# johanngerberding/voxelnet-pytorch

Measured on AMD Instinct MI355X. Metric: point-clouds/sec fwd+bwd, KITTI car voxel grid, batch=2, higher is better.
Workload: dtype bf16; 1 GPU; KITTI car config (voxel 0.2x0.2x0.4 m, grid 10x400x352, T=35), batch=2 per GPU, fwd+bwd train step (BASELINE configs[1]); global_batch=2, points_per_frame=19861, parallelism=dp1, launch_mode=eager+native-executor+one-call-step

## Files before the change

include/voxelnet_hip.h:

```cpp
#ifndef VOXELNET_HIP_H
#define VOXELNET_HIP_H

#include <stddef.h>
#include <stdint.h>

#ifdef __cplusplus
extern "C" {
#endif

#define VN_OK 0
#define VN_EINVAL (-1)
#define VN_EUNSUPPORTED (-2)
#define VN_EWORKSPACE (-3)

typedef enum { VN_F32 = 0, VN_BF16 = 1,
               VN_F32X3 = 2,
               VN_F32X3S = 3 } vnDtype;

typedef void *vnStream;

int vn_abi_version(void);
const char *vn_build_info(void);
const char *vn_build_id(void);

// ... 72 lines not shown
    int32_t Dr, Hr, Wr;
    int32_t Cs;
    int32_t src_wrap;
    int32_t Cr;
    int32_t kD, kH, kW;
    int32_t mulD, mulH, mulW;
    int32_t tmulD, tmulH, tmulW;
    int32_t padD, padH, padW;
    int32_t divD, divH, divW;
    int64_t src_sB, src_sD, src_sH, src_sW;
    int64_t out_sB, out_sD, out_sH, out_sW;
} vnConv;

int64_t vn_conv_stats_slab_rows(const vnConv *geom);
int vn_conv_gather_gemm(const void *src, const void *w_packed ,
                        const float *bias , void *out, vnDtype out_dtype,
                        const vnConv *geom, int32_t accumulate, float *stats_slab,
                        vnStream stream);
int32_t vn_conv_plan_id(const vnConv *geom);

size_t vn_conv_wgrad_workspace_bytes(const vnConv *geom, int32_t split, int64_t n_rows);
int vn_conv_wgrad(const void *src , const void *rows , float *dw_packed,
                  const vnConv *geom, int32_t split, void *workspace, size_t workspace_bytes,
                  vnStream stream);
int32_t vn_conv_wgrad_plan_id(const vnConv *geom, int32_t split, int64_t n_rows);
int vn_conv_wgrad_partials(const void *src, const void *rows, const vnConv *geom, int32_t split,
                           const int64_t *row_list, int64_t n_rows, void *workspace,
                           size_t workspace_bytes, int32_t *chunks, vnStream stream);
int vn_conv_wgrad_partials_split_pass(const void *src, const void *rows, const vnConv *geom, int32_t pass, void *workspace,
                                      size_t workspace_bytes, int32_t *chunks, vnStream stream);

int vn_conv_dgrad_bn_bwd(const void *src, const void *w_packed, void *out, vnDtype out_dtype, const vnConv *geom,
                         const void *bn_y, vnDtype bn_y_dtype, const float *bn_stats, float *slab, vnStream stream);
int vn_conv_gather_gemm_rows(const void *src, const void *w_packed, const float *bias, void *out,
                             vnDtype out_dtype, const vnConv *geom, const int64_t *row_list,
                             int64_t row_cap, const int32_t *row_count, int32_t out_linear,
                             float *stats_slab, vnStream stream);
int vn_conv_wgrad_rows(const void *src, const void *rows, float *dw_packed, const vnConv *geom,
                       const int64_t *row_list, int64_t n_rows, void *workspace, size_t workspace_bytes,
                       vnStream stream);
int vn_conv_wgrad_partials_counted(const void *src, const void *rows, const vnConv *geom, const int64_t *row_list,
                                   int64_t row_cap, const int32_t *row_count, void *workspace, size_t workspace_bytes,
                                   int32_t *chunks, vnStream stream);
size_t vn_active_sites_workspace_bytes(const vnConv *geom);
int vn_active_sites(const int64_t *coord, int64_t K, const vnConv *geom, void *workspace,
                    size_t workspace_bytes, int64_t *list, int64_t cap, int32_t *count, vnStream stream);
int vn_voxel_index_grid(const int64_t *coord, int64_t K, int32_t B, int32_t D, int32_t H, int32_t W,
                        int32_t *grid , vnStream stream);
int64_t vn_rulebook_slab_rows(int64_t cap);
int vn_rulebook_combine(const float *P, const int32_t *index_grid, const int64_t *list, int64_t cap,
                        const int32_t *count, const vnConv *geom, const float *bias, void *y,
                        vnDtype y_dtype, float *stats_slab, vnStream stream);
int vn_fill_rows(void *y, vnDtype dtype, int64_t M, int32_t C, int64_t stride, const float *values,
                 vnStream stream);

int vn_pack_weight(const float *w, int32_t c_out, int32_t c_in, int32_t taps, int32_t mode,
                   int32_t split3, int32_t cin_fold, void *packed, vnDtype packed_dtype,
                   vnStream stream);
int vn_unpack_wgrad(const float *dw_packed, int32_t c_out, int32_t c_in, int32_t taps,
                    int32_t mode, int32_t cin_fold, float *dw, vnStream stream);
typedef struct vnPackJob {
    const float *w;
    void *packed;
    int32_t c_out, c_in, taps, mode, split3, cin_fold;
    int32_t packed_dtype;
    int32_t pad_;
// ... 474 lines not shown
```

voxelnet-pytorch_amd/csrc/abi.hip:

```cpp
#include "common.h"
#include <mutex>
#include <stdio.h>
#include <stdlib.h>
#include <string.h>

#include "build_id.h"

extern "C" int vn_abi_version(void) { return 4; }
extern "C" const char *vn_build_id(void) { return VN_BUILD_ID; }

namespace {
const char *const KNOBS[] = {"VN_DUP", "VN_EARLY_DECONV", "VN_FUSE_BWD_REDUCE", "VN_GG_CONFIG", "VN_HEADS_STREAM", "VN_M0_BN", "VN_PATCH", "VN_PATCH2D",
                               "VN_SKIP", "VN_WGP_BLOCKS", "VN_WGRAD_PATCH", "VN_WG_BLOCKS"};
constexpr int NKNOBS = sizeof(KNOBS) / sizeof(KNOBS[0]);
}

int vn_knob(const char *name, int dflt) {
    for (int i = 0; i < NKNOBS; ++i)
        if (!strcmp(KNOBS[i], name)) {
            const char *e = getenv(name);
            return e && *e ? atoi(e) : dflt;
        }
    static std::mutex mu;
    static const char *seen[16];
    static int nseen = 0;
    std::lock_guard<std::mutex> lock(mu);
    for (int i = 0; i < nseen; ++i)
        if (!strcmp(seen[i], name)) return dflt;
    if (nseen < 16) seen[nseen++] = name;
    fprintf(stderr, "libvoxelnet_hip: vn_knob(\"%s\") is not in the KNOBS table of csrc/abi.hip — the default %d is used and the "
                    "environment is NOT read\n", name, dflt);
    return dflt;
}

extern "C" const char *vn_build_info(void) {
    static char buf[1536];
    static std::once_flag once;
    std::call_once(once, [] {
        size_t n = (size_t)snprintf(buf, sizeof(buf), "libvoxelnet_hip gfx950 (CDNA4) abi %d build " VN_BUILD_ID " " __DATE__ " " __TIME__, vn_abi_version());
        bool any = false;
        for (int i = 0; i < NKNOBS && n + 64 < sizeof(buf); ++i) {
            const char *e = getenv(KNOBS[i]);
            if (!e || !*e) continue;
            n += (size_t)snprintf(buf + n, sizeof(buf) - n, "%s%s=%.24s", any ? " " : " overrides: ", KNOBS[i], e);
            any = true;
        }
// ... 4 lines not shown
```

voxelnet-pytorch_amd/csrc/conv.hip:

```cpp
#include "common.h"

namespace {

constexpr int GG_MAX_TAPS = 32;
constexpr int GG_MAX_CLASSES = 16;
constexpr uint32_t GG_OOB = 0xFFFFF000u;
constexpr uint32_t GG_MAX_WINDOW = 0xFFFFE000u;

struct GGClass {
    int32_t tap_begin, ntaps;
    int32_t nD, nH, nW;
    int32_t qD, qH, qW;
    int32_t ooffD, ooffH, ooffW;
    int32_t offD[4], offH[4], offW[4];
};
struct GGTap {
    int32_t id, ih, iw, widx;
};
struct GGParams {
    const char *src;
    const char *w;
    const float *bias;
    char *out;
    float *stats;
// ... 873 lines not shown
                            acc[i][j] = __builtin_amdgcn_mfma_f32_16x16x32_bf16(a, bq[j], acc[i][j], 0, 0, 0);
                    }
                }
            }
            }
#ifdef VN_P2D_TRACE
            if (tr_on) {
                asm volatile("s_nop 0" ::"v"(acc[0][0]), "v"(acc[SM - 1][3]));
                P2D_STAMP(s, 4);
            }
#endif
        }
        pbuf ^= 1;
    }

    __syncthreads();
    int32_t *otab = reinterpret_cast<int32_t *>(smem);
    for (int r = threadIdx.x; r < BM; r += NT) {
        const int py = r / TW, px = r - py * TW;
        const int qh = y0 + py, qw = x0 + px;
        int32_t off = -1;
        if (qh < cl.qH && qw < cl.qW) {
            const int od = qd * p.omulD + cl.ooffD, oh = qh * p.omulH + cl.ooffH, ow = qw * p.omulW + cl.ooffW;
            if (od < p.Do && oh < p.Ho && ow < p.Wo)
                off = (int32_t)((int64_t)b * p.oB + (int64_t)od * p.oD + (int64_t)oh * p.oH + (int64_t)ow * p.oW);
        }
        otab[r] = off;
    }
    __syncthreads();
    if (p.bn_y) gg_store<WM, WN, SM, true>(p, acc, smem, otab, tile, n0, wm, wn, lane);
    else gg_store<WM, WN, SM>(p, acc, smem, otab, tile, n0, wm, wn, lane);
}

inline int floordiv(int a, int b) { return (a >= 0) ? a / b : -((-a + b - 1) / b); }
inline int posmod(int a, int b) { int r = a % b; return r < 0 ? r + b : r; }

struct AxisClass {
    int r;
    int q;
    int n;
    int tap[4];
    int off[4];
};

int axis_classes(int R, int k, int mul, int tmul, int pad, int div, AxisClass *out, int *mul_out, int *omul_out) {
    if (div == 1) {
        AxisClass c{};
        c.r = 0; c.q = R; c.n = k;
        for (int t = 0; t < k; ++t) { c.tap[t] = t; c.off[t] = t * tmul - pad; }
        out[0] = c;
        *mul_out = mul; *omul_out = 1;
        return 1;
    }
    int nc = 0;
    for (int r = 0; r < div && r < R; ++r) {
        AxisClass c{};
        c.r = r; c.q = (R - r + div - 1) / div; c.n = 0;
        for (int t = 0; t < k; ++t) {
            const int num = r + t * tmul - pad;
            if (posmod(num, div) == 0) { c.tap[c.n] = t; c.off[c.n] = floordiv(num, div); ++c.n; }
        }
        out[nc++] = c;
    }
    *mul_out = 1; *omul_out = div;
    return nc;
}
// ... 71 lines not shown
    constexpr size_t lds = 2 * ((size_t)((PROWS + 7) / 8 + NW - 1) / NW * NW * 1024) + NSB * (size_t)(64 * WN) * 128;
    static const hipError_t attr = hipFuncSetAttribute(reinterpret_cast<const void *>(&k_conv_patch2d<WM, WN, SM, TW, NSB, F32>),
                                                       hipFuncAttributeMaxDynamicSharedMemorySize, (int)lds);
    if (attr != hipSuccess) return (int)attr;
    k_conv_patch2d<WM, WN, SM, TW, NSB, F32><<<grid, 64 * NW, lds, st>>>(p);
    return 0;
}
int patch2d_stages() {
    static const int v = vn_knob("VN_PATCH2D", 3);
    return v;
}
int launch_patch_cfg(const PatchCfg &c, bool f32, const GGParams &p, dim3 grid, hipStream_t st) {
    if (c.id == 2 && p.Ds == 1 && p.nclasses == 1 && p.cls[0].nD == 1 && patch2d_stages() >= 3) {
        const GGParams &q = p;
        if (patch2d_stages() == 3 && !f32) return launch_patch2d<4, 2, 1, 16, 3, false>(q, grid, st);
        if (patch2d_stages() == 3 && f32 && q.x3) return launch_patch2d<4, 2, 1, 16, 3, true>(q, grid, st);
        if (patch2d_stages() == 3)
            return f32 ? launch_patch2d<2, 2, 2, 16, 3, true>(q, grid, st) : launch_patch2d<2, 2, 2, 16, 3, false>(q, grid, st);
        return f32 ? launch_patch2d<2, 2, 2, 16, 4, true>(q, grid, st) : launch_patch2d<2, 2, 2, 16, 4, false>(q, grid, st);
    }
    if (c.id == 3) return f32 ? launch_patch<4, 1, 3, 32, true>(p, grid, st) : launch_patch<4, 1, 3, 32, false>(p, grid, st);
    if (c.id == 2) return f32 ? launch_patch<2, 2, 2, 16, true>(p, grid, st) : launch_patch<2, 2, 2, 16, false>(p, grid, st);
    return f32 ? launch_patch<2, 2, 5, 16, true>(p, grid, st) : launch_patch<2, 2, 5, 16, false>(p, grid, st);
}

int launch_cfg(const GGConfig &c, bool f32, const GGParams &p, dim3 grid, hipStream_t st) {
    switch (c.id) {
    case 0: return f32 ? launch_gg<4, 1, 4, 2, true>(p, grid, st) : launch_gg<4, 1, 4, 2, false>(p, grid, st);
    case 1: return f32 ? launch_gg<2, 2, 4, 2, true>(p, grid, st) : launch_gg<2, 2, 4, 2, false>(p, grid, st);
    case 2: return f32 ? launch_gg<2, 2, 2, 4, true>(p, grid, st) : launch_gg<2, 2, 2, 4, false>(p, grid, st);
    case 3: return f32 ? launch_gg<4, 1, 1, 6, true>(p, grid, st) : launch_gg<4, 1, 1, 6, false>(p, grid, st);
    default: return f32 ? launch_gg<2, 2, 5, 2, true>(p, grid, st) : launch_gg<2, 2, 5, 2, false>(p, grid, st);
    }
}

struct AxisSlots {
    int n, cls[4], off[4], tap[4];
};
bool axis_slots(int k, int tmul, int pad, int div, AxisSlots *o) {
    o->n = 0;
    for (int r = 0; r < div; ++r)
        for (int t = 0; t < k; ++t) {
            const int num = r + t * tmul - pad;
            if (posmod(num, div) != 0) continue;
            if (o->n >= 4) return false;
            o->cls[o->n] = div == 1 ? -1 : r;
            o->off[o->n] = floordiv(num, div);
            o->tap[o->n] = t;
            ++o->n;
        }
    return o->n > 0;
}

}

extern "C" int vn_conv_gather_gemm_rows(const void *src, const void *w_packed, const float *bias, void *out,
                                        vnDtype out_dtype, const vnConv *g, const int64_t *row_list, int64_t row_cap,
                                        const int32_t *row_count, int32_t out_linear, float *stats_slab,
                                        vnStream stream) {
    VN_CHECK_ARG(src && w_packed && out && g && row_list && row_cap >= 0 && row_cap < (1ll << 31));
    if (row_cap == 0) return VN_OK;
    VN_CHECK_ARG(g->B > 0 && g->Ds > 0 && g->Hs > 0 && g->Ws > 0 && g->Dr > 0 && g->Hr > 0 && g->Wr > 0);
    VN_CHECK_ARG(g->kD >= 1 && g->kD <= 4 && g->kH >= 1 && g->kH <= 4 && g->kW >= 1 && g->kW <= 4);
    VN_CHECK_ARG(g->divD >= 1 && g->divH >= 1 && g->divW >= 1);
    VN_CHECK_ARG((g->divD == 1 || g->mulD == 1) && (g->divH == 1 || g->mulH == 1) && (g->divW == 1 || g->mulW == 1));
    VN_CHECK_ARG(out_dtype == VN_F32 || out_dtype == VN_BF16);
// ... 91 lines not shown
    const int64_t rows = (int64_t)g->B * g->Dr * g->Hr * g->Wr;
    return vn_ceil_div(rows, gg_config(rows, g->Cr, 1).BM);
}

extern "C" int32_t vn_conv_plan_id(const vnConv *g) {
    if (!g || g->divD < 1 || g->divH < 1 || g->divW < 1 || g->B <= 0) return -1;
    const PatchCfg pc = patch_config(g);
    if (pc.id == 2 && g->Ds == 1 && g->Dr == 1 && g->kD == 1 && g->divD == 1 && patch2d_stages() >= 3)
        return 120 + patch2d_stages();
    if (pc.id >= 0) return 100 + pc.id;
    const int64_t qd = vn_ceil_div(g->Dr, g->divD), qh = vn_ceil_div(g->Hr, g->divH), qw = vn_ceil_div(g->Wr, g->divW);
    const int nd = g->divD < g->Dr ? g->divD : g->Dr, nh = g->divH < g->Hr ? g->divH : g->Hr, nw = g->divW < g->Wr ? g->divW : g->Wr;
    return gg_config((int64_t)g->B * qd * qh * qw, g->Cr, nd * nh * nw).id;
}

static int gather_gemm_impl(const void *src, const void *w_packed, const float *bias, void *out, vnDtype out_dtype,
                            const vnConv *g, int32_t accumulate, float *stats_slab, vnStream stream, const void *bn_y,
                            vnDtype bn_y_dtype, const float *bn_stats);

extern "C" int vn_conv_gather_gemm(const void *src, const void *w_packed, const float *bias, void *out,
                                   vnDtype out_dtype, const vnConv *g, int32_t accumulate, float *stats_slab,
                                   vnStream stream) {
    return gather_gemm_impl(src, w_packed, bias, out, out_dtype, g, accumulate, stats_slab, stream, nullptr, VN_BF16, nullptr);
}

extern "C" int vn_conv_dgrad_bn_bwd(const void *src, const void *w_packed, void *out, vnDtype out_dtype, const vnConv *g,
                                    const void *bn_y, vnDtype bn_y_dtype, const float *bn_stats, float *slab,
                                    vnStream stream) {
    VN_CHECK_ARG(bn_y && bn_stats && slab && g);
    if (vn_conv_plan_id(g) != 123) return VN_EUNSUPPORTED;
    return gather_gemm_impl(src, w_packed, nullptr, out, out_dtype, g, 0, slab, stream, bn_y, bn_y_dtype, bn_stats);
}

static int gather_gemm_impl(const void *src, const void *w_packed, const float *bias, void *out, vnDtype out_dtype,
                            const vnConv *g, int32_t accumulate, float *stats_slab, vnStream stream, const void *bn_y,
                            vnDtype bn_y_dtype, const float *bn_stats) {
    VN_CHECK_ARG(src && w_packed && out && g);
    VN_CHECK_ARG(g->B > 0 && g->Ds > 0 && g->Hs > 0 && g->Ws > 0 && g->Dr > 0 && g->Hr > 0 && g->Wr > 0);
    VN_CHECK_ARG(g->kD >= 1 && g->kD <= 4 && g->kH >= 1 && g->kH <= 4 && g->kW >= 1 && g->kW <= 4);
    VN_CHECK_ARG(g->kD * g->kH * g->kW <= GG_MAX_TAPS);
    VN_CHECK_ARG(g->divD >= 1 && g->divH >= 1 && g->divW >= 1);
    VN_CHECK_ARG(g->divD == 1 || g->mulD == 1);
    VN_CHECK_ARG(g->divH == 1 || g->mulH == 1);
    VN_CHECK_ARG(g->divW == 1 || g->mulW == 1);
    VN_CHECK_ARG(out_dtype == VN_F32 || out_dtype == VN_BF16);
    VN_CHECK_ARG(!stats_slab || g->divD * g->divH * g->divW <= GG_MAX_CLASSES);
    VN_CHECK_ARG(g->dtype == VN_BF16 || g->dtype == VN_F32 || g->dtype == VN_F32X3 || g->dtype == VN_F32X3S);
    const bool f32 = g->dtype != VN_BF16;
    const int esz = f32 ? 4 : 2, bke = 128 / esz, align_e = 16 / esz;
    (void)bke;
    if (g->Cs <= 0 || (g->Cs % align_e) || g->Cr <= 0 || (g->Cr & 3)) return VN_EUNSUPPORTED;
    if (g->src_wrap != 0) return VN_EUNSUPPORTED;
    if (g->divD * g->divH * g->divW > GG_MAX_CLASSES) return VN_EUNSUPPORTED;
    if (((g->src_sB | g->src_sD | g->src_sH | g->src_sW) & (align_e - 1)) != 0) return VN_EUNSUPPORTED;
    if (((g->out_sB | g->out_sD | g->out_sH | g->out_sW) & 3) != 0) return VN_EUNSUPPORTED;
    if ((reinterpret_cast<uintptr_t>(src) & 15) || (reinterpret_cast<uintptr_t>(w_packed) & 15) ||
        (reinterpret_cast<uintptr_t>(out) & 15))
        return VN_EUNSUPPORTED;

    GGParams p{};
    p.src = static_cast<const char *>(src);
    p.w = static_cast<const char *>(w_packed);
    p.bias = bias;
    p.out = static_cast<char *>(out);
    p.stats = stats_slab;
    p.bn_y = bn_y;
// ... 106 lines not shown
```

voxelnet-pytorch_amd/csrc/runtime.hip:

```cpp
#include "common.h"
#include <new>
#include <string.h>

namespace {

constexpr int NL = 23;

struct Spec {
    int dim, cin, cout, k[3], s[3], p[3];
    bool transposed;
    int cin_fold;
};

struct Rows {
    char *ptr;
    int dtype;
    int B, D, H, W, C;
    int64_t sB, sD, sH, sW;
    int64_t M() const { return (int64_t)B * D * H * W; }
};

Rows dense_rows(void *ptr, int dtype, int B, int D, int H, int W, int C, int64_t width = 0) {
    if (!width) width = C;
    return Rows{static_cast<char *>(ptr), dtype, B, D, H, W, C, (int64_t)D * H * W * width, (int64_t)H * W * width,
// ... 1011 lines not shown
                vn_dgrad_total(dy.ptr, (vnDtype)dy.dtype, B, P.odims[l][0], P.odims[l][1], P.odims[l][2], C, sp.cin, sp.k[0],
                               L[l].weight, 0, P.dtot_ws, P.dtot_ws_bytes, P.dtot, bs));
            if (box_on_side) {
                box_ev = net->next_event();
                if (!box_ev) return VN_EINVAL;
                VN_HIP(hipEventRecord(box_ev, ws));
            }
            const int64_t rs[4] = {0, 0, 0, sp.cin};
            vnConv gl = geom(dy, P.in_dims[l], C, sp.cin, sp.k, ONE, NEG, np, sp.s, rs);
            RTT(T_CONV_DGRAD, l, 2.0 * active_rows * taps * sp.cin * C, rows_bytes(dy) + 2.0 * active_rows * sp.cin * P.esz, ls,
                vn_conv_gather_gemm_rows(dy.ptr, P.wp_d[l], nullptr, P.dx[l].ptr, (vnDtype)P.dx[l].dtype, cx(P, gl), P.alist, P.acap,
                                         P.acount, 1, nullptr, ls));
            return VN_OK;
        }
        Rows dx = P.dx[l];
        if (l == 0) {
            if (!d_input) return VN_OK;
            dx = dense_rows(d_input, P.adt, B, cfg->D, cfg->H, cfg->W, 128);
        }
        const int64_t os[4] = {dx.sB, dx.sD, dx.sH, dx.sW};
        vnConv gd = sp.transposed ? geom(dy, P.in_dims[l], C, sp.cin, sp.k, sp.s, ONE, sp.p, ONE, os)
                                  : geom(dy, P.in_dims[l], C, sp.cin, sp.k, ONE, NEG, np, sp.s, os);
        const bool below_plain = l >= 2 && l - 1 != L_M2 && l - 1 != L_D1 && l - 1 != L_D2 && l - 1 != L_D3 && l != L_D1 &&
                                 l != L_D2 && l != L_D3 && !P.spec[l - 1].transposed;
        if (fuse_bwd_reduce_on() && single_call && !accumulate && !on_side && below_plain && vn_conv_plan_id(cx(P, gd)) == 123 &&
            P.y[l - 1].sB == dx.sB && P.y[l - 1].sD == dx.sD && P.y[l - 1].sH == dx.sH && P.y[l - 1].sW == dx.sW &&
            vn_conv_stats_slab_rows(cx(P, gd)) <= P.bslab_rows[l - 1]) {
            RTT(T_CONV_DGRAD, l, layer_flops(sp, P.in_dims[l], P.odims[l], B), rows_bytes(dy) + 2.0 * rows_bytes(dx), ls,
                vn_conv_dgrad_bn_bwd(dy.ptr, P.wp_d[l], dx.ptr, (vnDtype)dx.dtype, cx(P, gd), P.y[l - 1].ptr, (vnDtype)P.y[l - 1].dtype,
                                     P.stats[l - 1], P.bslab[l - 1], ls));
            fused_rows[l - 1] = vn_conv_stats_slab_rows(cx(P, gd));
            return VN_OK;
        }
        RTT(T_CONV_DGRAD, l, layer_flops(sp, P.in_dims[l], P.odims[l], B), rows_bytes(dy) + rows_bytes(dx), ls,
            vn_conv_gather_gemm(dy.ptr, P.wp_d[l], nullptr, dx.ptr, (vnDtype)dx.dtype, cx(P, gd), accumulate ? 1 : 0, nullptr, ls));
        return VN_OK;
    };
    static const int early_on = vn_knob("VN_EARLY_DECONV", 1);
    const bool early = early_on && ws != hs && seg_begin == 0 && seg_end == NL + 1;
    hipEvent_t ev_d2 = nullptr, ev_d1 = nullptr;
    if (early) {
        if (!heads_forked) RT(fork());
        RT(do_layer(L_D2, wstream, true, false));
        ev_d2 = net->next_event();
        if (!ev_d2) return VN_EINVAL;
        VN_HIP(hipEventRecord(ev_d2, ws));
        RT(do_layer(L_D1, wstream, true, false));
        ev_d1 = net->next_event();
        if (!ev_d1) return VN_EINVAL;
        VN_HIP(hipEventRecord(ev_d1, ws));
    }
    const bool bucket_ev = cfg->bucket_events && ws != hs && seg_begin == 0 && seg_end == NL + 1;
    int u_done = 0, z_done = 0;
    auto bucket_done = [&](int b) -> int {
        RT(flush());
            if (b == 3 && m0_on_main) RT(fork());
        RTT(T_UNPACK, -1, 0.0, unpack_bytes(unpack + u_done, nu - u_done), wstream, vn_unpack_wgrads_batch(unpack + u_done, nu - u_done, wstream));
        RT(after_unpack(u_done, nu, wstream));
        u_done = nu;
        if (zj.n > z_done) {
            ZeroJobs part{};
            part.n = zj.n - z_done;
            for (int i = 0; i < part.n; ++i) { part.ptr[i] = zj.ptr[z_done + i]; part.len[i] = zj.len[z_done + i]; }
            RTT(T_MISC, -1, 0.0, 0.0, wstream, zero_many(part, ws));
            z_done = zj.n;
        }
// ... 145 lines not shown
```

voxelnet-pytorch_amd/voxelnet_amd/_lib.py:

```python
import ctypes
import os

import torch

_HERE = os.path.dirname(os.path.abspath(__file__))
LIB_PATH = os.environ.get("VN_LIB_PATH") or os.path.join(_HERE, "lib", "libvoxelnet_hip.so")

c_i32, c_i64, c_f32, c_vp, c_sz = ctypes.c_int32, ctypes.c_int64, ctypes.c_float, ctypes.c_void_p, ctypes.c_size_t

VN_F32, VN_BF16 = 0, 1
VN_F32X3S = 3


class VnGrid(ctypes.Structure):
    _fields_ = [("D", c_i32), ("H", c_i32), ("W", c_i32),
                ("vz", c_f32), ("vy", c_f32), ("vx", c_f32),
                ("ox", c_f32), ("oy", c_f32), ("oz", c_f32), ("T", c_i32)]


class VnConv(ctypes.Structure):
    _fields_ = [(n, c_i32) for n in (
        "dtype", "B", "Ds", "Hs", "Ws", "Dr", "Hr", "Wr", "Cs", "src_wrap", "Cr", "kD", "kH", "kW",
        "mulD", "mulH", "mulW", "tmulD", "tmulH", "tmulW", "padD", "padH", "padW",
        "divD", "divH", "divW")] + [(n, c_i64) for n in (
# ... 162 lines not shown
    "vn_vfe_workspace_bytes": (c_sz, [c_i64, c_i32]),
    "vn_vfe_fwd": (c_i32, [c_vp, c_i64, c_i32, _P(VnVfeWeights), c_i32, c_f32, c_f32, c_vp, c_vp, c_vp, c_sz, c_vp]),
    "vn_vfe_fwd_rows": (c_i32, [c_vp, c_i64, c_i32, _P(VnVfeWeights), c_i32, c_f32, c_f32, c_vp, c_vp, c_vp, c_vp, c_sz, c_vp]),
    "vn_vfe_bwd": (c_i32, [c_vp, c_i64, c_i32, _P(VnVfeWeights), c_vp, c_vp, _P(VnVfeGrads), c_vp, c_sz, c_i32, c_vp]),
    "vn_scatter_dense_fwd": (c_i32, [c_vp, c_vp, c_i64, c_i32, c_i32, c_i32, c_i32, c_i32, c_vp, c_i32, c_i32,
                                     c_i32, c_vp]),
    "vn_scatter_dense_update": (c_i32, [c_vp, c_vp, c_i64, c_i32, c_i32, c_i32, c_i32, c_i32, c_vp, c_i32, c_i32,
                                        c_i32, c_vp]),
    "vn_scatter_dense_bwd": (c_i32, [c_vp, c_i32, c_vp, c_i64, c_i32, c_i32, c_i32, c_i32, c_i32, c_vp, c_vp]),
    "vn_conv_gather_gemm": (c_i32, [c_vp, c_vp, c_vp, c_vp, c_i32, _P(VnConv), c_i32, c_vp, c_vp]),
    "vn_net_workspace_bytes": (c_sz, [_P(VnNetConfig), c_i64]),
    "vn_net_tensor_info": (c_i32, [_P(VnNetConfig), c_i64, c_i32, c_i32, _P(VnNetTensorInfo)]),
    "vn_net_create": (c_i32, [_P(c_vp)]),
    "vn_net_destroy": (c_i32, [c_vp]),
    "vn_net_step": (c_i32, [c_vp, _P(VnNetConfig), _P(VnStep)]),
    "vn_net_timing_begin": (c_i32, [c_vp, c_i32]),
    "vn_net_timing_read": (c_i32, [c_vp, c_vp, c_i32, _P(c_i32)]),
    "vn_net_forward": (c_i32, [c_vp, _P(VnNetConfig), _P(VnLayerParams), c_vp, c_vp, c_vp, c_vp, c_vp, c_i64, c_vp, c_sz, c_vp,
                               c_vp, c_vp, c_vp]),
    "vn_net_wait_bucket": (c_i32, [c_vp, c_i32, c_vp]),
    "vn_net_prepare": (c_i32, [c_vp, _P(VnNetConfig), _P(VnLayerParams), c_vp, c_vp, c_i64, c_vp, c_sz, c_vp]),
    "vn_voxel_index_grid": (c_i32, [c_vp, c_i64, c_i32, c_i32, c_i32, c_i32, c_vp, c_vp]),
    "vn_rulebook_slab_rows": (c_i64, [c_i64]),
    "vn_rulebook_combine": (c_i32, [c_vp, c_vp, c_vp, c_i64, c_vp, _P(VnConv), c_vp, c_vp, c_i32, c_vp, c_vp]),
    "vn_net_backward": (c_i32, [c_vp, _P(VnNetConfig), _P(VnLayerParams), c_vp, c_vp, c_vp, c_vp, c_vp, c_vp, c_vp, c_i64,
                                c_vp, c_sz, _P(VnLayerGrads), c_vp, c_vp, c_vp, c_i32, c_i32, c_vp, c_vp]),
    "vn_conv_stats_slab_rows": (c_i64, [_P(VnConv)]),
    "vn_conv_plan_id": (c_i32, [_P(VnConv)]),
    "vn_conv_wgrad_plan_id": (c_i32, [_P(VnConv), c_i32, c_i64]),
    "vn_bn_finalize_slab": (c_i32, [c_vp, c_i64, c_i64, c_i32, c_vp, c_vp, c_vp, c_vp, c_vp, c_f32, c_f32, c_vp, c_vp]),
    "vn_conv_wgrad_workspace_bytes": (c_sz, [_P(VnConv), c_i32, c_i64]),
    "vn_conv_wgrad": (c_i32, [c_vp, c_vp, c_vp, _P(VnConv), c_i32, c_vp, c_sz, c_vp]),
    "vn_conv_dgrad_bn_bwd": (c_i32, [c_vp, c_vp, c_vp, c_i32, _P(VnConv), c_vp, c_i32, c_vp, c_vp, c_vp]),
    "vn_conv_gather_gemm_rows": (c_i32, [c_vp, c_vp, c_vp, c_vp, c_i32, _P(VnConv), c_vp, c_i64, c_vp, c_i32, c_vp, c_vp]),
    "vn_conv_wgrad_partials": (c_i32, [c_vp, c_vp, _P(VnConv), c_i32, c_vp, c_i64, c_vp, c_sz, c_vp, c_vp]),
    "vn_conv_wgrad_rows": (c_i32, [c_vp, c_vp, c_vp, _P(VnConv), c_vp, c_i64, c_vp, c_sz, c_vp]),
    "vn_conv_wgrad_partials_split_pass": (c_i32, [c_vp, c_vp, _P(VnConv), c_i32, c_vp, c_sz, c_vp, c_vp]),
    "vn_active_sites_workspace_bytes": (c_sz, [_P(VnConv)]),
    "vn_active_sites": (c_i32, [c_vp, c_i64, _P(VnConv), c_vp, c_sz, c_vp, c_i64, c_vp, c_vp]),
    "vn_fill_rows": (c_i32, [c_vp, c_i32, c_i64, c_i32, c_i64, c_vp, c_vp]),
    "vn_pack_weight": (c_i32, [c_vp, c_i32, c_i32, c_i32, c_i32, c_i32, c_i32, c_vp, c_i32, c_vp]),
    "vn_unpack_wgrad": (c_i32, [c_vp, c_i32, c_i32, c_i32, c_i32, c_i32, c_vp, c_vp]),
    "vn_bn_stats": (c_i32, [c_vp, c_i32, c_i64, c_i32, c_i64, c_i32, c_vp, c_vp, c_vp]),
    "vn_bn_finalize": (c_i32, [c_vp, c_i64, c_i32, c_i32, c_vp, c_vp, c_vp, c_vp, c_vp, c_i32, c_f32, c_f32, c_vp,
                               c_vp]),
    "vn_bn_apply": (c_i32, [c_vp, c_i32, c_i64, c_i64, c_i32, c_vp, c_i32, c_vp, c_i32, c_i64, c_i64, c_vp]),
    "vn_bn_bwd_reduce": (c_i32, [c_vp, c_i32, c_i64, c_vp, c_i32, c_i64, c_i64, c_i32, c_vp, c_i32, c_vp, c_vp]),
    "vn_bn_bwd_finalize": (c_i32, [c_vp, c_i64, c_i32, c_i32, c_vp, c_vp, c_vp, c_vp, c_vp, c_vp]),
    "vn_bn_bwd_slab_rows": (c_i64, [c_i64, c_i32]),
    "vn_bn_bwd_reduce_slab": (c_i32, [c_vp, c_i32, c_i64, c_vp, c_i32, c_i64, c_i64, c_i32, c_vp, c_i32, c_vp, c_vp]),
    "vn_bn_bwd_finalize_slab": (c_i32, [c_vp, c_i64, c_i64, c_i32, c_vp, c_vp, c_vp, c_vp, c_vp, c_vp]),
    "vn_bn_bwd_apply": (c_i32, [c_vp, c_i32, c_i64, c_vp, c_i32, c_i64, c_i64, c_i32, c_vp, c_vp, c_i32, c_vp,
                                c_i32, c_i64, c_i64, c_vp]),
    "vn_bn_apply_bev": (c_i32, [c_vp, c_i32, c_i64, c_i32, c_i64, c_vp, c_i32, c_vp, c_i32, c_i64, c_vp]),
    "vn_bn_bwd_reduce_slab_bev": (c_i32, [c_vp, c_i32, c_i64, c_vp, c_i32, c_i64, c_i32, c_i64, c_vp, c_i32, c_vp, c_vp]),
    "vn_bn_bwd_apply_bev": (c_i32, [c_vp, c_i32, c_i64, c_vp, c_i32, c_i64, c_i32, c_i64, c_vp, c_vp, c_i32, c_vp, c_i32, c_vp]),
    "vn_bn_apply_flagged": (c_i32, [c_vp, c_i32, c_i64, c_i64, c_i32, c_vp, c_i32, c_vp, c_i32, c_i64, c_vp, c_vp, c_vp]),
    "vn_bn_bwd_reduce_slab_flagged": (c_i32, [c_vp, c_i32, c_i64, c_vp, c_i32, c_i64, c_i64, c_i32, c_vp, c_i32, c_vp, c_vp, c_vp,
                                              c_vp]),
    "vn_bn_bwd_apply_list": (c_i32, [c_vp, c_i32, c_vp, c_i32, c_i32, c_i32, c_i32, c_i32, c_vp, c_vp, c_i32, c_vp, c_i32, c_vp,
                                     c_vp, c_i64, c_vp]),
    "vn_bn_bwd_list_slab_rows": (c_i64, [c_i64, c_i32]),
    "vn_bn_bwd_reduce_list": (c_i32, [c_vp, c_i32, c_vp, c_i32, c_i32, c_i32, c_i32, c_i32, c_vp, c_i32, c_vp, c_vp, c_vp, c_i64, c_vp]),
    "vn_bn_bwd_finalize_list": (c_i32, [c_vp, c_i64, c_i64, c_i32, c_vp, c_vp, c_vp, c_vp, c_i32, c_i32, c_vp, c_vp, c_vp, c_vp]),
    "vn_bn_bwd_apply_list_rows": (c_i32, [c_vp, c_i32, c_vp, c_i32, c_i32, c_i32, c_i32, c_i32, c_vp, c_vp, c_i32, c_vp, c_i32,
                                          c_vp, c_vp, c_i64, c_vp]),
# ... 172 lines not shown
```

Measured before the change: 572.5 point-clouds/s.

## Add patch-based dgrad kernel for stride-2 3x3 convs sharing one input patch

Adds a dedicated dgrad kernel for stride-2 3x3 2D convolutions. It stages one (TH+1)x(TW+1) patch of dy into LDS per channel chunk and computes all four output parity classes from it, with separate accumulators per class. Weights are pipelined through three LDS stages, and taps are scheduled round-robin across classes. This replaces the generic gather-GEMM path, which handled each parity class separately and re-read dy for each one, so the aim is to cut redundant global loads and launches. In exchange it adds larger LDS use, more accumulator registers, and a hand-written wait/barrier schedule that must stay correct.

```diff
diff --git a/include/voxelnet_hip.h b/include/voxelnet_hip.h
--- a/include/voxelnet_hip.h
+++ b/include/voxelnet_hip.h
@@ -128,6 +128,9 @@
 
 int vn_conv_dgrad_bn_bwd(const void *src, const void *w_packed, void *out, vnDtype out_dtype, const vnConv *geom,
                          const void *bn_y, vnDtype bn_y_dtype, const float *bn_stats, float *slab, vnStream stream);
+int vn_conv_s2_dgrad(const void *dy, const void *w_packed, void *dx, vnDtype out_dtype, const vnConv *geom,
+                     int32_t accumulate, int32_t tile_rows, vnStream stream);
+int32_t vn_conv_s2_plan_id(const vnConv *geom);
 int vn_conv_gather_gemm_rows(const void *src, const void *w_packed, const float *bias, void *out,
                              vnDtype out_dtype, const vnConv *geom, const int64_t *row_list,
                              int64_t row_cap, const int32_t *row_count, int32_t out_linear,
diff --git a/voxelnet-pytorch_amd/csrc/abi.hip b/voxelnet-pytorch_amd/csrc/abi.hip
--- a/voxelnet-pytorch_amd/csrc/abi.hip
+++ b/voxelnet-pytorch_amd/csrc/abi.hip
@@ -11,7 +11,7 @@
 
 namespace {
 const char *const KNOBS[] = {"VN_DUP", "VN_EARLY_DECONV", "VN_FUSE_BWD_REDUCE", "VN_GG_CONFIG", "VN_HEADS_STREAM", "VN_M0_BN", "VN_PATCH", "VN_PATCH2D",
-                               "VN_SKIP", "VN_WGP_BLOCKS", "VN_WGRAD_PATCH", "VN_WG_BLOCKS"};
+                               "VN_S2_PATCH", "VN_SKIP", "VN_WGP_BLOCKS", "VN_WGRAD_PATCH", "VN_WG_BLOCKS"};
 constexpr int NKNOBS = sizeof(KNOBS) / sizeof(KNOBS[0]);
 }
 
diff --git a/voxelnet-pytorch_amd/csrc/conv.hip b/voxelnet-pytorch_amd/csrc/conv.hip
--- a/voxelnet-pytorch_amd/csrc/conv.hip
+++ b/voxelnet-pytorch_amd/csrc/conv.hip
@@ -929,6 +929,160 @@
     else gg_store<WM, WN, SM>(p, acc, smem, otab, tile, n0, wm, wn, lane);
 }
 
+struct S2Sched {
+    int tap[36], kc[36];
+};
+constexpr S2Sched s2_sched(int nk) {
+    constexpr int CLS_TAPS[4][4] = {{4, -1, -1, -1}, {3, 5, -1, -1}, {1, 7, -1, -1}, {0, 2, 6, 8}};
+    S2Sched r{};
+    int n = 0;
+    for (int round = 0; round < 4; ++round)
+        for (int kc = 0; kc < nk; ++kc)
+            for (int c = 0; c < 4; ++c)
+                if (CLS_TAPS[c][round] >= 0) { r.tap[n] = CLS_TAPS[c][round]; r.kc[n] = kc; ++n; }
+    return r;
+}
+template <int WM, int WN, int TW, int NSB, int NK>
+__global__ void __launch_bounds__(64 * WM * WN) k_s2_dgrad_patch(const GGParams p) {
+    VN_PRIO_MAIN();
+    constexpr int NW = WM * WN, NT = 64 * NW;
+    constexpr int BM = 16 * WM, BN = 64 * WN, TH = BM / TW;
+    static_assert((NW == 4 || NW == 8) && BM % TW == 0 && (BN / 8) % NW == 0, "4 or 8 waves; whole patch lines");
+    constexpr int PW = TW + 1, PH = TH + 1, PROWS = PH * PW;
+    constexpr int PPIECES = (PROWS + 7) / 8;
+    constexpr int PA = (PPIECES + NW - 1) / NW;
+    constexpr int PATCH_BYTES = PA * NW * 1024;
+    constexpr int RB = BN / (8 * NW);
+    constexpr int B_BYTES = BN * 128;
+    static_assert(NSB == 3 && RB <= 63, "the waits below are written for three weight stages");
+    static_assert(4 * BM * 4 <= PATCH_BYTES, "the epilogue's four offset tables reuse the first patch buffer");
+    extern __shared__ __attribute__((aligned(16))) char smem[];
+    char *bst = smem + NK * PATCH_BYTES;
+
+    const int lane = threadIdx.x & 63;
+    const int wave = __builtin_amdgcn_readfirstlane(threadIdx.x >> 6);
+    const int wm = wave / WN, wn = wave % WN;
+    const int ntn = (p.N + BN - 1) / BN;
+    int bid = blockIdx.x;
+    {
+        const int nwg = gridDim.x, q = nwg >> 3, r = nwg & 7, x = bid & 7;
+        bid = (x < r ? x * (q + 1) : r * (q + 1) + (x - r) * q) + (bid >> 3);
+    }
+    const int tile = bid / ntn, tile_n = bid - tile * ntn;
+    const int n0 = tile_n * BN;
+    const int tiles_x = (p.Ws + TW - 1) / TW, tiles_y = (p.Hs + TH - 1) / TH;
+    int t = tile;
+    const int tx = t % tiles_x; t /= tiles_x;
+    const int ty = t % tiles_y;
+    const int b = t / tiles_y;
+    if (b >= p.B) return;
+    const int y0 = ty * TH, x0 = tx * TW;
+
+    const int a_chunk = (lane & 7) ^ ((wave * 4 + (lane >> 4)) & 7);
+    uint32_t a_row[PA];
+#pragma unroll
+    for (int i = 0; i < PA; ++i) {
+        const int q = (i * NW + wave) * 8 + (lane >> 3);
+        const int qy = q / PW, qx = q - qy * PW;
+        const int sy = y0 + qy, sx = x0 + qx;
+        a_row[i] = (q < PROWS && sy < p.Hs && sx < p.Ws) ? (uint32_t)(((int64_t)sy * p.sH + (int64_t)sx * p.sW) * 2) : GG_OOB;
+    }
+    uint32_t b_row[RB];
+#pragma unroll
+    for (int i = 0; i < RB; ++i) {
+        const int rho = (i * NW + wave) * 8 + (lane >> 3);
+        const int rl = rho & 63;
+        const int n = n0 + (rho & ~63) + (rl & 15) * 4 + (rl >> 4);
+        b_row[i] = n < p.N ? (uint32_t)((int64_t)n * p.Cs * 2) : GG_OOB;
+    }
+    const char *src_base = p.src + (int64_t)b * p.sB * 2;
+    const __amdgpu_buffer_rsrc_t rs_a = vn_uniform_rsrc(src_base, (uint32_t)(p.src_batch_extent * 2));
+    const __amdgpu_buffer_rsrc_t rs_b = vn_uniform_rsrc(p.w, p.w_bytes);
+    const int k_lane0 = a_chunk * 8;
+
+    const int fr = lane & 15, fq = lane >> 4;
+    int q0;
+    {
+        const int r = wm * 16 + fr;
+        const int py = r / TW, px = r - py * TW;
+        q0 = py * PW + px;
+    }
+    const int bfrag0 = fr * 128 + (((0 + fq) ^ (fr >> 1)) << 4);
+    const int bfrag1 = fr * 128 + (((4 + fq) ^ (fr >> 1)) << 4);
+
+    f32x4_t acc[4][1][4];
+#pragma unroll
+    for (int c = 0; c < 4; ++c)
+#pragma unroll
+        for (int j = 0; j < 4; ++j) acc[c][0][j] = f32x4_t{0.f, 0.f, 0.f, 0.f};
+
+    const uint32_t tap_bytes = (uint32_t)p.N * (uint32_t)p.Cs * 2u;
+    auto stage_b = [&](int tap, int kc, int buf) {
+        const int k_lane = kc * 64 + k_lane0;
+        const bool k_ok = k_lane < p.Cs;
+        const uint32_t b_koff = (uint32_t)k_lane * 2u;
+        const uint32_t b_soff = __builtin_amdgcn_readfirstlane((uint32_t)tap * tap_bytes);
+        char *lb = bst + buf * B_BYTES + wave * 1024;
+#pragma unroll
+        for (int i = 0; i < RB; ++i)
+            lds_dma16(rs_b, lb + i * (NW * 1024), (k_ok && b_row[i] != GG_OOB) ? b_row[i] + b_koff : GG_OOB, b_soff);
+    };
+    auto stage_patch = [&](int kc, char *patch) {
+        const int k_lane = kc * 64 + k_lane0;
+        const bool k_ok = k_lane < p.Cs;
+        const uint32_t off = (uint32_t)k_lane * 2u;
+#pragma unroll
+        for (int i = 0; i < PA; ++i)
+            lds_dma16(rs_a, patch + (i * NW + wave) * 1024, (k_ok && a_row[i] != GG_OOB) ? a_row[i] + off : GG_OOB, 0);
+    };
+
+    constexpr S2Sched SCH = s2_sched(NK);
+    constexpr int total = NK * 9;
+    stage_patch(0, smem);
+#pragma unroll
+    for (int s = 0; s < NSB - 1; ++s) stage_b(SCH.tap[s], SCH.kc[s], s);
+#pragma unroll
+    for (int s = 0; s < total; ++s) {
+        if (total - 1 - s >= 1) asm volatile("s_waitcnt vmcnt(%0) lgkmcnt(0)" ::"n"(RB) : "memory");
+        else asm volatile("s_waitcnt vmcnt(0) lgkmcnt(0)" ::: "memory");
+        __builtin_amdgcn_s_barrier();
+        asm volatile("" ::: "memory");
+        if (s % 4 == 1 && s / 4 + 1 < NK) stage_patch(s / 4 + 1, smem + (s / 4 + 1) * PATCH_BYTES);
+        if (s + NSB - 1 < total) stage_b(SCH.tap[s + NSB - 1], SCH.kc[s + NSB - 1], (s + NSB - 1) % NSB);
+        const int tap = SCH.tap[s], kh = tap / 3, kw = tap - kh * 3;
+        const int cls = (kh != 1 ? 2 : 0) + (kw != 1 ? 1 : 0);
+        const int q = q0 + (kh == 0 ? PW : 0) + (kw == 0 ? 1 : 0);
+        const char *patch = smem + SCH.kc[s] * PATCH_BYTES;
+        const char *lb = bst + (s % NSB) * B_BYTES + wn * (64 * 128);
+#pragma unroll
+        for (int ks = 0; ks < 2; ++ks) {
+            const int fo = ks ? bfrag1 : bfrag0;
+            bf16x8_t bq[4];
+#pragma unroll
+            for (int j = 0; j < 4; ++j) bq[j] = *reinterpret_cast<const bf16x8_t *>(lb + j * 2048 + fo);
+            const bf16x8_t a = *reinterpret_cast<const bf16x8_t *>(patch + q * 128 + (((ks * 4 + fq) ^ ((q >> 1) & 7)) << 4));
+#pragma unroll
+            for (int j = 0; j < 4; ++j)
+                acc[cls][0][j] = __builtin_amdgcn_mfma_f32_16x16x32_bf16(a, bq[j], acc[cls][0][j], 0, 0, 0);
+        }
+    }
+
+    __syncthreads();
+    int32_t *otab = reinterpret_cast<int32_t *>(smem);
+    for (int i = threadIdx.x; i < 4 * BM; i += NT) {
+        const int c = i / BM, r = i - c * BM;
+        const int py = r / TW, px = r - py * TW;
+        const int ch = y0 + py, cw = x0 + px;
+        const int oh = 2 * ch + (c >> 1), ow = 2 * cw + (c & 1);
+        otab[i] = (ch < p.Hs && cw < p.Ws && oh < p.Ho && ow < p.Wo)
+                      ? (int32_t)((int64_t)b * p.oB + (int64_t)oh * p.oH + (int64_t)ow * p.oW)
+                      : -1;
+    }
+    __syncthreads();
+#pragma unroll
+    for (int c = 0; c < 4; ++c) gg_store<WM, WN, 1>(p, acc[c], smem, otab + c * BM, 0, n0, wm, wn, lane);
+}
+
 inline int floordiv(int a, int b) { return (a >= 0) ? a / b : -((-a + b - 1) / b); }
 inline int posmod(int a, int b) { int r = a % b; return r < 0 ? r + b : r; }
 
@@ -1066,6 +1220,38 @@
     case 3: return f32 ? launch_gg<4, 1, 1, 6, true>(p, grid, st) : launch_gg<4, 1, 1, 6, false>(p, grid, st);
     default: return f32 ? launch_gg<2, 2, 5, 2, true>(p, grid, st) : launch_gg<2, 2, 5, 2, false>(p, grid, st);
     }
+}
+
+int s2_patch_enabled() {
+    static const int v = vn_knob("VN_S2_PATCH", 1);
+    return v;
+}
+bool s2_dgrad_geom(const vnConv *g) {
+    if (g->dtype != VN_BF16 || g->B <= 0 || g->src_wrap != 0) return false;
+    if (g->Ds != 1 || g->Dr != 1 || g->kD != 1 || g->mulD != 1 || g->padD != 0 || g->divD != 1) return false;
+    if (g->kH != 3 || g->kW != 3 || g->mulH != 1 || g->mulW != 1 || g->tmulH != -1 || g->tmulW != -1) return false;
+    if (g->padH != -1 || g->padW != -1 || g->divH != 2 || g->divW != 2) return false;
+    if (g->Hr <= 0 || g->Wr <= 0 || g->Hs != (g->Hr - 1) / 2 + 1 || g->Ws != (g->Wr - 1) / 2 + 1) return false;
+    if (!((g->Cs == 128 || g->Cs == 256) && g->Cr > 0 && (g->Cr & 3) == 0)) return false;
+    if (((g->src_sB | g->src_sH | g->src_sW) & 7) != 0 || ((g->out_sB | g->out_sH | g->out_sW) & 3) != 0) return false;
+    if (g->src_sH < 0 || g->src_sW < 0 || g->out_sB < 0 || g->out_sH < 0 || g->out_sW < 0) return false;
+    if ((int64_t)9 * g->Cr * g->Cs * 2 > (int64_t)GG_MAX_WINDOW) return false;
+    const int64_t src_extent = (int64_t)(g->Hs - 1) * g->src_sH + (int64_t)(g->Ws - 1) * g->src_sW + g->Cs;
+    if (src_extent * 2 > (int64_t)GG_MAX_WINDOW - 4096) return false;
+    const int64_t out_extent = (int64_t)(g->B - 1) * g->out_sB + (int64_t)(g->Hr - 1) * g->out_sH + (int64_t)(g->Wr - 1) * g->out_sW + g->Cr;
+    if (out_extent >= (1ll << 31)) return false;
+    return (int64_t)g->B * vn_ceil_div(g->Hs, 2) * vn_ceil_div(g->Ws, 16) * vn_ceil_div(g->Cr, 128) <= 0x7fffffffll;
+}
+int s2_dgrad_tile_rows(const vnConv *g) { return g->Cs == 128 ? 4 : 2; }
+template <int WM, int WN, int TW, int NSB, int NK>
+int launch_s2_dgrad(const GGParams &p, int64_t tiles, hipStream_t st) {
+    constexpr int NW = WM * WN, TH = 16 * WM / TW, PROWS = (TH + 1) * (TW + 1);
+    constexpr size_t lds = NK * ((size_t)((PROWS + 7) / 8 + NW - 1) / NW * NW * 1024) + NSB * (size_t)(64 * WN) * 128;
+    static const hipError_t attr = hipFuncSetAttribute(reinterpret_cast<const void *>(&k_s2_dgrad_patch<WM, WN, TW, NSB, NK>),
+                                                       hipFuncAttributeMaxDynamicSharedMemorySize, (int)lds);
+    if (attr != hipSuccess) return (int)attr;
+    k_s2_dgrad_patch<WM, WN, TW, NSB, NK><<<dim3((unsigned)tiles), 64 * NW, lds, st>>>(p);
+    return 0;
 }
 
 struct AxisSlots {
@@ -1223,6 +1409,46 @@
     return gather_gemm_impl(src, w_packed, nullptr, out, out_dtype, g, 0, slab, stream, bn_y, bn_y_dtype, bn_stats);
 }
 
+extern "C" int32_t vn_conv_s2_plan_id(const vnConv *g) {
+    if (!g || !s2_patch_enabled()) return 0;
+    return s2_dgrad_geom(g) ? 1 : 0;
+}
+
+extern "C" int vn_conv_s2_dgrad(const void *dy, const void *w_packed, void *dx, vnDtype out_dtype, const vnConv *g,
+                                int32_t accumulate, int32_t tile_rows, vnStream stream) {
+    VN_CHECK_ARG(dy && w_packed && dx && g);
+    VN_CHECK_ARG(out_dtype == VN_F32 || out_dtype == VN_BF16);
+    VN_CHECK_ARG(tile_rows == 0 || tile_rows == 2 || tile_rows == 4);
+    if (!s2_dgrad_geom(g)) return VN_EUNSUPPORTED;
+    if (tile_rows == 4 && g->Cs != 128) return VN_EUNSUPPORTED;
+    if ((reinterpret_cast<uintptr_t>(dy) & 15) || (reinterpret_cast<uintptr_t>(w_packed) & 15) || (reinterpret_cast<uintptr_t>(dx) & 15))
+        return VN_EUNSUPPORTED;
+    GGParams p{};
+    p.src = static_cast<const char *>(dy);
+    p.w = static_cast<const char *>(w_packed);
+    p.out = static_cast<char *>(dx);
+    p.sB = g->src_sB; p.sH = g->src_sH; p.sW = g->src_sW;
+    p.oB = g->out_sB; p.oH = g->out_sH; p.oW = g->out_sW;
+    p.B = g->B; p.Ds = 1; p.Hs = g->Hs; p.Ws = g->Ws;
+    p.Do = 1; p.Ho = g->Hr; p.Wo = g->Wr;
+    p.Cs = g->Cs; p.N = g->Cr;
+    p.out_f32 = out_dtype == VN_F32;
+    p.accumulate = accumulate ? 1 : 0;
+    p.src_row_elems = g->Cs;
+    p.esz = 2;
+    p.w_bytes = (uint32_t)((int64_t)9 * g->Cr * g->Cs * 2);
+    p.src_batch_extent = (int64_t)(g->Hs - 1) * g->src_sH + (int64_t)(g->Ws - 1) * g->src_sW + g->Cs;
+    const int th = tile_rows ? tile_rows : s2_dgrad_tile_rows(g);
+    const int64_t tiles = (int64_t)g->B * vn_ceil_div(g->Hs, th) * vn_ceil_div(g->Ws, 16) * vn_ceil_div(g->Cr, 128);
+    hipStream_t st = vn_stream(stream);
+    int rc;
+    if (g->Cs == 128) rc = th == 4 ? launch_s2_dgrad<4, 2, 16, 3, 2>(p, tiles, st) : launch_s2_dgrad<2, 2, 16, 3, 2>(p, tiles, st);
+    else rc = launch_s2_dgrad<2, 2, 16, 3, 4>(p, tiles, st);
+    if (rc) return rc;
+    VN_LAUNCH_STATUS();
+    return VN_OK;
+}
+
 static int gather_gemm_impl(const void *src, const void *w_packed, const float *bias, void *out, vnDtype out_dtype,
                             const vnConv *g, int32_t accumulate, float *stats_slab, vnStream stream, const void *bn_y,
                             vnDtype bn_y_dtype, const float *bn_stats) {
diff --git a/voxelnet-pytorch_amd/csrc/runtime.hip b/voxelnet-pytorch_amd/csrc/runtime.hip
--- a/voxelnet-pytorch_amd/csrc/runtime.hip
+++ b/voxelnet-pytorch_amd/csrc/runtime.hip
@@ -1067,6 +1067,11 @@
             fused_rows[l - 1] = vn_conv_stats_slab_rows(cx(P, gd));
             return VN_OK;
         }
+        if (vn_conv_s2_plan_id(cx(P, gd)) == 1) {
+            RTT(T_CONV_DGRAD, l, layer_flops(sp, P.in_dims[l], P.odims[l], B), rows_bytes(dy) + rows_bytes(dx), ls,
+                vn_conv_s2_dgrad(dy.ptr, P.wp_d[l], dx.ptr, (vnDtype)dx.dtype, cx(P, gd), accumulate ? 1 : 0, 0, ls));
+            return VN_OK;
+        }
         RTT(T_CONV_DGRAD, l, layer_flops(sp, P.in_dims[l], P.odims[l], B), rows_bytes(dy) + rows_bytes(dx), ls,
             vn_conv_gather_gemm(dy.ptr, P.wp_d[l], nullptr, dx.ptr, (vnDtype)dx.dtype, cx(P, gd), accumulate ? 1 : 0, nullptr, ls));
         return VN_OK;
diff --git a/voxelnet-pytorch_amd/voxelnet_amd/_lib.py b/voxelnet-pytorch_amd/voxelnet_amd/_lib.py
--- a/voxelnet-pytorch_amd/voxelnet_amd/_lib.py
+++ b/voxelnet-pytorch_amd/voxelnet_amd/_lib.py
@@ -218,6 +218,8 @@
     "vn_conv_wgrad_workspace_bytes": (c_sz, [_P(VnConv), c_i32, c_i64]),
     "vn_conv_wgrad": (c_i32, [c_vp, c_vp, c_vp, _P(VnConv), c_i32, c_vp, c_sz, c_vp]),
     "vn_conv_dgrad_bn_bwd": (c_i32, [c_vp, c_vp, c_vp, c_i32, _P(VnConv), c_vp, c_i32, c_vp, c_vp, c_vp]),
+    "vn_conv_s2_dgrad": (c_i32, [c_vp, c_vp, c_vp, c_i32, _P(VnConv), c_i32, c_i32, c_vp]),
+    "vn_conv_s2_plan_id": (c_i32, [_P(VnConv)]),
     "vn_conv_gather_gemm_rows": (c_i32, [c_vp, c_vp, c_vp, c_vp, c_i32, _P(VnConv), c_vp, c_i64, c_vp, c_i32, c_vp, c_vp]),
     "vn_conv_wgrad_partials": (c_i32, [c_vp, c_vp, _P(VnConv), c_i32, c_vp, c_i64, c_vp, c_sz, c_vp, c_vp]),
     "vn_conv_wgrad_rows": (c_i32, [c_vp, c_vp, c_vp, _P(VnConv), c_vp, c_i64, c_vp, c_sz, c_vp]),
```

Result: no change. 577.2 point-clouds/s (median of 6 runs) (+0.8%).
